# ChenWu98/cycle-diffusion

Measured on NVIDIA H100. Metric: images/sec (512x512, 50-step encode+decode) at 1/2/4/8 H100; ms/U-Net-call, higher is better.
Workload: dtype fp32

## Files before the change

cycle_diffusion_b200/_cabi.py:

```python
import ctypes as C
import os

HERE = os.path.dirname(os.path.abspath(__file__))
LIB_PATH = os.path.join(HERE, 'libcdx.so')

CDX_UNET_OPENAI = 1
CDX_UNET_IDDPM = 2
CDX_UNET_DDPM = 3
CDX_TEXT_OPENCLIP = 4
CDX_PRED_EPS = 0
CDX_PRED_V = 1


class UnetConfig(C.Structure):
    _fields_ = [('kind', C.c_int), ('in_channels', C.c_int), ('out_channels', C.c_int), ('model_channels', C.c_int),
                ('num_res_blocks', C.c_int), ('n_mult', C.c_int), ('channel_mult', C.c_int * 8), ('n_attn', C.c_int),
                ('attention_ds', C.c_int * 8), ('num_heads', C.c_int), ('num_head_channels', C.c_int),
                ('context_dim', C.c_int)]


class VaeConfig(C.Structure):
    _fields_ = [('ch', C.c_int), ('n_mult', C.c_int), ('ch_mult', C.c_int * 8), ('num_res_blocks', C.c_int),
                ('in_channels', C.c_int), ('out_ch', C.c_int), ('z_channels', C.c_int), ('embed_dim', C.c_int), ('vq', C.c_int), ('n_embed', C.c_int)]

# ... 99 lines not shown

class SemanticAttnMaskC(C.Structure):
    _fields_ = [('intersect', C.c_int), ('n_tokens', C.c_int * CDX_SEMANTIC_MAX)]


class LocalBlendC(C.Structure):
    _fields_ = [('alpha_src', C.c_void_p), ('alpha_tgt', C.c_void_p), ('sub_src', C.c_void_p), ('sub_tgt', C.c_void_p), ('start_step', C.c_int),
                ('th_blend', C.c_float), ('th_sub', C.c_float)]


_F = C.c_float
_I = C.c_int
_S = C.c_size_t

SIGNATURES = {
    'cdx_abi_version': (_I, []),
    'cdx_last_error': (C.c_char_p, []),
    'cdx_engine_create': (_I, [_I, C.POINTER(_P)]),
    'cdx_engine_destroy': (None, [_P]),
    'cdx_engine_workspace_bytes': (_S, [_P]),
    'cdx_engine_launch_count': (C.c_uint64, [_P]),
    'cdx_engine_set_mma_mode': (_I, [_P, _I]),
    'cdx_engine_set_persist': (_I, [_P, _I, _I]),
    'cdx_engine_profile': (_I, [_P, _I]),
    'cdx_engine_profile_read': (_I, [_P, _I, C.POINTER(C.c_double), C.POINTER(C.c_double), C.POINTER(C.c_double), C.POINTER(C.c_uint64)]),
    'cdx_unet_create': (_I, [_P, C.POINTER(UnetConfig), C.POINTER(_P)]),
    'cdx_vae_create': (_I, [_P, C.POINTER(VaeConfig), C.POINTER(_P)]),
    'cdx_text_create': (_I, [_P, C.POINTER(TextConfig), C.POINTER(_P)]),
    'cdx_net_destroy': (None, [_P]),
    'cdx_net_num_params': (_I, [_P]),
    'cdx_net_param_name': (C.c_char_p, [_P, _I]),
    'cdx_net_param_shape': (_I, [_P, _I, C.POINTER(C.c_int64)]),
    'cdx_net_load_param': (_I, [_P, C.c_char_p, _P, _I, C.POINTER(C.c_int64), _I]),
    'cdx_net_finalize': (_I, [_P]),
    'cdx_net_weight_blob': (_I, [_P, C.POINTER(_P), C.POINTER(_S)]),
    'cdx_net_adopt_blob': (_I, [_P]),
    'cdx_unet_set_time_freqs': (_I, [_P, C.POINTER(_F), _I]),
    'cdx_unet_set_prediction': (_I, [_P, _I, C.POINTER(_F), C.POINTER(_F), _I]),
    'cdx_unet_forward': (_I, [_P, _P, _P, _P, _I, _P, _I, _I, _I, _P]),
    'cdx_vae_encode': (_I, [_P, _P, _P, _I, _I, _P]),
    'cdx_text_encode': (_I, [_P, _P, _I, _I, _P, _P]),
    'cdx_vae_decode': (_I, [_P, _P, _P, _I, _I, _P]),
    'cdx_vae_encode_hw': (_I, [_P, _P, _P, _I, _I, _I, _P]),
    'cdx_vae_decode_hw': (_I, [_P, _P, _P, _I, _I, _I, _P]),
    'cdx_affine': (_I, [_P, _P, _F, _F, _P, _S, _P]),
    'cdx_shift_scale': (_I, [_P, _P, _F, _F, _P, _S, _P]),
# ... 108 lines not shown
```

cycle_diffusion_b200/csrc/cabi.cu:

```cuda
#include <stdio.h>
#include <stdlib.h>
#include <string.h>

#include <algorithm>

#include "nets.cuh"

struct cdx_engine { cdx::Engine e; };
struct cdx_net { cdx::Net* n; cdx_engine* owner; };

namespace cdx {
const std::string& last_error();

namespace {

template <class F>
int guard(F&& f) {
  try {
    f();
    return CDX_OK;
  } catch (const Error& err) {
    set_last_error(err.what());
    return err.code;
  } catch (const std::exception& err) {
// ... 569 lines not shown

int cdx_abi_version(void) { return CDX_ABI_VERSION; }
const char* cdx_last_error(void) { return cdx::last_error().c_str(); }

int cdx_engine_create(int device, cdx_engine** out) {
  return guard([&] {
    CDX_CHECK(out != nullptr, "engine_create: null out");
    int count = 0;
    cudaError_t err = cudaGetDeviceCount(&count);
    if (err != cudaSuccess || count <= 0)
      throw Error(CDX_E_CUDA, std::string("no usable CUDA device (there is no CPU fallback): ") + cudaGetErrorString(err));
    CDX_CHECK(device >= 0 && device < count, "engine_create: device %d out of range (count %d)", device, count);
    CDX_CUDA(cudaSetDevice(device));
    cudaDeviceProp prop;
    CDX_CUDA(cudaGetDeviceProperties(&prop, device));
    cdx_engine* eng = new cdx_engine();
    eng->e.device = device;
    if (prop.major != 9 || prop.minor != 0)
      throw Error(CDX_E_CUDA, "libcdx is built for sm_90a (H100) only; device " + std::to_string(device) + " is sm_" +
                                  std::to_string(prop.major) + std::to_string(prop.minor));
    eng->e.num_sms = prop.multiProcessorCount;
    const char* persist = getenv("CDX_PERSIST");
    eng->e.persist = persist == nullptr || atoi(persist) != 0;
    *out = eng;
  });
}
void cdx_engine_destroy(cdx_engine* e) {
  if (!e) return;
  cudaSetDevice(e->e.device);
  cudaDeviceSynchronize();
  e->e.arena.destroy();
  if (e->e.done_ev) cudaEventDestroy(e->e.done_ev);
  if (e->e.side) cudaStreamDestroy(e->e.side);
  if (e->e.fork_ev) cudaEventDestroy(e->e.fork_ev);
  if (e->e.join_ev) cudaEventDestroy(e->e.join_ev);
  if (e->e.amax_pool) cudaFree(e->e.amax_pool);
  delete e;
}
size_t cdx_engine_workspace_bytes(const cdx_engine* e) { return e ? e->e.arena.cap : 0; }
uint64_t cdx_engine_launch_count(const cdx_engine* e) { return e ? e->e.launches : 0; }
int cdx_engine_set_mma_mode(cdx_engine* e, int mode) {
  return guard([&] {
    CDX_CHECK(e != nullptr && mode >= 0 && mode <= 5, "set_mma_mode: bad arguments");
    e->e.mma_mode = mode == 0 ? 0 : 1;
    e->e.flash_attn = mode != 2 && mode != 0;
    e->e.tc_kind = mode == 3 ? 0 : mode >= 4 ? 2 : 1;
    e->e.attn_one = mode == 5;
  });
}

int cdx_engine_set_persist(cdx_engine* e, int enable, int max_ctas) {
  return guard([&] {
    CDX_CHECK(e != nullptr && max_ctas >= 0, "set_persist: bad arguments");
    e->e.persist = enable != 0;
    e->e.persist_grid = max_ctas;
  });
}

int cdx_engine_profile(cdx_engine* e, int enable) {
  return guard([&] {
    CDX_CHECK(e != nullptr, "profile: null engine");
    CDX_CUDA(cudaSetDevice(e->e.device));
    CDX_CUDA(cudaDeviceSynchronize());
    for (ProfRec& r : e->e.prof.recs) { cudaEventDestroy(r.a); cudaEventDestroy(r.b); }
    e->e.prof.recs.clear();
    e->e.prof.on = enable != 0;
  });
}
int cdx_engine_profile_read(cdx_engine* e, int tag, double* ms, double* flops, double* bytes, uint64_t* launches) {
  return guard([&] {
    CDX_CHECK(e && ms && flops && bytes && launches && tag >= 0 && tag < PROF_NTAGS, "profile_read: bad arguments");
    CDX_CUDA(cudaSetDevice(e->e.device));
    CDX_CUDA(cudaDeviceSynchronize());
    *ms = 0; *flops = 0; *bytes = 0; *launches = 0;
    const bool dump = getenv("CDX_PROF_DUMP") != nullptr;
    for (const ProfRec& r : e->e.prof.recs) {
      if (r.tag != tag) continue;
      float t = 0.f;
// ... 1226 lines not shown
```

cycle_diffusion_b200/csrc/common.cuh:

```cuda
#pragma once
#include <cuda_runtime.h>
#include <stdint.h>
#include <stdio.h>
#include <string>
#include <vector>
#include <stdexcept>

#include "../../include/cdx.h"

namespace cdx {

struct Error : std::runtime_error {
  int code;
  Error(int c, const std::string& m) : std::runtime_error(m), code(c) {}
};
void set_last_error(const std::string& m);

#define CDX_CHECK(cond, ...)                                                     \
  do {                                                                           \
    if (!(cond)) {                                                               \
      char _b[512];                                                              \
      snprintf(_b, sizeof(_b), __VA_ARGS__);                                     \
      throw ::cdx::Error(CDX_E_INVALID, std::string(_b) + " [" #cond "]");       \
    }                                                                            \
// ... 22 lines not shown
};

enum ProfTag {
  PROF_CONV_FFMA = 0, PROF_DENSE_FFMA = 1, PROF_BATCHED_FFMA = 2, PROF_CONV_TC = 3, PROF_DENSE_TC = 4, PROF_BATCHED_TC = 5,
  PROF_GROUPNORM = 6, PROF_LAYERNORM = 7, PROF_SOFTMAX = 8, PROF_ELEMENTWISE = 9, PROF_NTAGS = 10
};
struct ProfRec { cudaEvent_t a, b; int tag; double flops, bytes; int launches; char note[56]; };
struct Profiler {
  bool on = false;
  std::vector<ProfRec> recs;
  std::vector<cudaEvent_t> pool;
};

struct Engine {
  Profiler prof;
  int device = 0;
  int num_sms = 132;
  bool flash_attn = true;
  int mma_mode = 1;
  int tc_kind = 1;
  bool attn_one = false;
  bool persist = true;
  int persist_grid = 0;
  float* amax_pool = nullptr;
  int amax_cap = 1 << 15, amax_used = 0, amax_high = 0;
  float* amax_slot();
  double* stat_pool = nullptr;
  size_t stat_cap = (size_t)8 << 20, stat_used = 0, stat_high = 0;
  size_t stat_dry = 0;
  double* stat_alloc(size_t n);
  void pools_reset(cudaStream_t s);
  Arena arena;
  cudaStream_t last_stream = nullptr;
  cudaEvent_t done_ev = nullptr;
  bool ev_recorded = false;
  cudaStream_t side = nullptr;
  cudaEvent_t fork_ev = nullptr, join_ev = nullptr;
  uint64_t launches = 0;
  bool dry() const { return arena.dry; }
};

struct ProfScope {
  Engine& e;
  cudaStream_t s;
  int idx = -1;
  ProfScope(Engine& eng, cudaStream_t st, int tag, double flops, double bytes, int launches);
// ... 32 lines not shown
  const float* Bw = nullptr; int ldb = 0; int b_kn = 0;
  const float* Bw_hi = nullptr; const float* Bw_lo = nullptr;
  const void* Bw_h_hi = nullptr; const void* Bw_h_lo = nullptr; int b_exp = 0;
  const float* a_amax = nullptr; const float* a2_amax = nullptr;
  float* c_amax = nullptr;
  double* c_stats = nullptr;
  float* Cout = nullptr; int ldc = 0;
  float* Cout_lo = nullptr;
  float* Ct_hi = nullptr; float* Ct_lo = nullptr; int t_col0 = 0; long long ldt = 0;
  const float* bias = nullptr;
  const float* rowvec = nullptr; int ld_rowvec = 0; int rows_per_batch = 1;
  const float* residual = nullptr; int ldr = 0;
  float alpha = 1.f;
  int geglu = 0;
  int out_nchw = 0;
  int rows_per_img = 0;
  int batch = 1, heads = 1;
  long long sA_b = 0, sA_h = 0, sB_b = 0, sB_h = 0, sC_b = 0, sC_h = 0;
};
void gemm(Engine& e, const GemmArgs& a, cudaStream_t s, int* route = nullptr);
bool gemm_tc(Engine& e, const GemmArgs& a, cudaStream_t s, int* side_done = nullptr);
enum { ROUTE_KIND_SS = 0, ROUTE_KIND_TS = 1, ROUTE_KIND_H16 = 2, ROUTE_KIND_H16_FAST = 3 };
inline int route_plan(int kind, int width, int splits) { return kind << 4 | width << 8 | splits << 16; }
bool flash_eligible(const Engine& e, int N, int Nk, int d, int C);
struct AttnPlanes {
  enum Fmt { TF32, H16 } fmt;
  const void* q_hi; const void* q_lo; int ldq;
  const void* k_hi; const void* k_lo; int ldk;
  const void* vt_hi; const void* vt_lo;
  const float* q_amax = nullptr; const float* k_amax = nullptr; const float* v_amax = nullptr;
};
bool flash_attention(Engine& e, const AttnPlanes& a, float* out, int ldo, int B, int N, int Nk, int Nks, int Nvs, int heads, int d, float scale,
                     cudaStream_t s, const int* qk_row = nullptr, const int* acc_rows = nullptr, int n_acc = 0, const int* kv_row = nullptr);
void split_rows_h16(Engine& e, const float* src, long long rows, int cols, long long ld, void* hi, void* lo, long long ldh, const float* amax,
                    cudaStream_t s);
void split_transpose_h16(Engine& e, const float* src, int R, int Cc, long long ld, void* hi, void* lo, const float* amax, cudaStream_t s,
                         int images = 1, int Rp = 0);
struct FlashPlan { int qrows, rag, ksplit, ring; };
FlashPlan flash_plan(int d, bool h16, bool one, int N);
bool self_attention_h16(Engine& e, const float* qkv, const float* slot, float* out, int B, int HW, int C, int heads, int d, float scale, bool lo,
                        cudaStream_t s, const int* qk_row, const int* kv_row, const int* acc_rows = nullptr, int n_acc = 0, int* Nvs_out = nullptr);
bool self_attention_tf32_padded(Engine& e, const float* qk_hi, const float* qk_lo, const float* vr, float* out, int B, int HW, int C, int heads,
                                int d, float scale, cudaStream_t s, const int* qk_row, const int* kv_row, const int* acc_rows = nullptr,
                                int n_acc = 0, int* Nvs_out = nullptr);
void context_split_h16(Engine& e, const float* kv, int Mk, int C, const float* slot, void* k_hi, void* k_lo, void* vt_hi, void* vt_lo,
                       cudaStream_t s);
// ... 127 lines not shown
```

cycle_diffusion_b200/csrc/kernels_tc.cu:

```cuda
#include <algorithm>

#include <mutex>
#include <array>
#include <map>
#include <unordered_map>
#include <vector>
#include <cstdlib>
#include <cmath>
#include <type_traits>

#include <cuda_fp16.h>

#include "tc_common.cuh"

namespace cdx {
namespace {

using namespace tc;

constexpr int TBM = 128, TBN = 128, TBK = 32;
constexpr int TILE_BYTES = TBM * TBK * 4;
constexpr int TC_THREADS = 384;
constexpr int SMEM_MAX = 232448;
constexpr int BAR_BYTES = 256, ALIGN_SLACK = 1024;
// ... 93 lines not shown
  } else {
    c.m0 = tm * TBM;
    c.zb = z / p.heads;
    c.zh = z - c.zb * p.heads;
  }
  return c;
}

__device__ __forceinline__ uint32_t tf32_lo(float x, uint32_t hi) { return rn_tf32(__float_as_uint(x - __uint_as_float(hi))); }

#ifdef CDX_GEMM_TIMELINE
constexpr int TL_SLOTS = 8;
__device__ unsigned long long* g_gemm_timeline = nullptr;
__device__ __forceinline__ void tl_stamp(int k) {
  unsigned long long t;
  asm volatile("mov.u64 %0, %%globaltimer;" : "=l"(t) :: "memory");
  if (g_gemm_timeline) g_gemm_timeline[(size_t)blockIdx.x * TL_SLOTS + k] = t;
}
#define TL_STAMP(k) tl_stamp(k)
#else
#define TL_STAMP(k) ((void)0)
#endif

template <int KIND, int BN, bool PERSIST = false>
__global__ void __launch_bounds__(TC_THREADS, 1)
tc_gemm_kernel(const __grid_constant__ CUtensorMap mapA, const __grid_constant__ CUtensorMap mapA2,
               const __grid_constant__ CUtensorMap mapB, const __grid_constant__ CUtensorMap mapBlo,
               const __grid_constant__ CUtensorMap mapR, const __grid_constant__ CUtensorMap mapC, const TcParams p) {
  using CF = Cfg<KIND, BN, PERSIST>;
  constexpr bool H16 = CF::H16, FAST = KIND == KIND_H16_FAST;
  constexpr int BK = CF::BK, KSTEPS = CF::KSTEPS, A_BYTES = CF::A_BYTES, B_PLANE = CF::B_PLANE, STAGE_BYTES = CF::STAGE_BYTES;
  constexpr int STAGES = CF::STAGES, EPI_BOX = CF::EPI_BOX, EPI_PER_SLOT = CF::EPI_PER_SLOT, EPI_SLOTS = CF::EPI_SLOTS;
  constexpr int NACC = BN / 2;
  if (threadIdx.x == 0) TL_STAMP(0);
  pdl_trigger();
  extern __shared__ uint8_t smem_raw[];
  const uint32_t base = (smem_u32(smem_raw) + 1023u) & ~1023u;
  const uint32_t epi = base + STAGES * STAGE_BYTES;
  const uint32_t bars = epi + CF::EPI_BYTES;
  auto bar_full = [&](int s) { return bars + 8u * s; };
  auto bar_empty = [&](int s) { return bars + 8u * (STAGES + s); };
  const uint32_t bar_res = bars + 16u * STAGES;
  const uint32_t bar_out = bar_res + 8u;

  const int warp = threadIdx.x >> 5, lane = threadIdx.x & 31;
  const int num_kb = (p.K + BK - 1) / BK;
  TileCoord tc_ = tile_coord(p, blockIdx.x, num_kb);
  int nst = tc_.kb1 - tc_.kb0;
  const bool staged = PERSIST || staged_store(p);
  auto epi_box = [&](int k) {
    return PERSIST ? epi + k * EPI_BOX : base + ((nst + k / EPI_PER_SLOT) % STAGES) * STAGE_BYTES + (k % EPI_PER_SLOT) * EPI_BOX;
  };

  if (threadIdx.x == 0) {
    for (int s = 0; s < STAGES; ++s) {
      mbar_init(bar_full(s), 1);
// ... 64 lines not shown
    asm volatile("setmaxnreg.dec.sync.aligned.u32 40;");
    if (threadIdx.x == 0) {
      const int cblocks = p.mode == 1 ? p.C1 / TBK : 0;
      int it = 0;
      for (int kb = tc_.kb0; kb < tc_.kb1; ++kb, ++it) {
        const int s = it % STAGES;
        mbar_wait(bar_empty(s), ((it / STAGES) & 1) ^ 1);
        const uint32_t st = base + s * STAGE_BYTES;
        const uint32_t sb = st + A_BYTES;
        const int k0 = kb * BK;
        if (p.mode == 2) {
          mbar_expect_tx(bar_full(s), TILE_BYTES + BN * 128);
          int ca[4], cb4[4];
#pragma unroll
          for (int i = 0; i < 4; ++i) {
            const int ac = p.a_code[i], bc = p.b_code[i];
            ca[i] = ac == 0 ? k0 : ac == 1 ? tc_.m0 + tc_.zh * p.a_rowoff_h : ac == 2 ? tc_.zh : ac == 3 ? tc_.zb : 0;
            cb4[i] = bc == 0 ? k0 : bc == 1 ? tc_.n0 + tc_.zh * p.b_rowoff_h : bc == 2 ? tc_.zh : bc == 3 ? tc_.zb : 0;
          }
          tma_load_4d(st, &mapA, ca[0], ca[1], ca[2], ca[3], bar_full(s));
          tma_load_4d(sb, &mapB, cb4[0], cb4[1], cb4[2], cb4[3], bar_full(s));
          continue;
        }
        mbar_expect_tx(bar_full(s), TILE_BYTES + (KIND == KIND_SS ? 1 : 2) * B_PLANE);
        if (p.mode == 0) {
          if (k0 < p.C1) tma_load_2d(st, &mapA, k0, tc_.m0, bar_full(s));
          else tma_load_2d(st, &mapA2, k0 - p.C1, tc_.m0, bar_full(s));
        } else {
          const int tap = kb / cblocks, cb = kb - tap * cblocks;
          const int dy = tap / 3, dx = tap - dy * 3;
          tma_load_4d(st, &mapA, cb * TBK, tc_.x0 * p.cstride + dx - p.cpad, tc_.y0 * p.cstride + dy - p.cpad, tc_.b0,
                      bar_full(s));
        }
        tma_load_2d(sb, &mapB, k0, tc_.n0, bar_full(s));
        if (KIND != KIND_SS) tma_load_2d(sb + B_PLANE, &mapBlo, k0, tc_.n0, bar_full(s));
      }
      if (staged) {
        if (p.residual) mbar_expect_tx(bar_res, BN * TBM * 4);
        for (int k = 0; k < EPI_SLOTS; ++k, ++it) {
          const int s = it % STAGES;
          mbar_wait(bar_empty(s), ((it / STAGES) & 1) ^ 1);
          if (!p.residual) continue;
          for (int b = k * EPI_PER_SLOT; b < min(BN / TBK, (k + 1) * EPI_PER_SLOT); ++b) {
            const uint32_t dst = epi_box(b);
            if (p.mode == 0) tma_load_2d(dst, &mapR, tc_.n0 + b * TBK, tc_.m0, bar_res);
            else tma_load_4d(dst, &mapR, tc_.n0 + b * TBK, tc_.x0, tc_.y0, tc_.b0, bar_res);
          }
        }
        if (!p.residual) mbar_arrive(bar_res);
      }
    }
    return;
  }

  asm volatile("setmaxnreg.inc.sync.aligned.u32 232;");
// ... 5 lines not shown
  float omax_cta = 0.f;
  int g0 = 0;
#pragma unroll 1
  for (int t = blockIdx.x, item = 0;;) {
    const int kchunk = (tc_.kb1 - tc_.kb0) <= 2 * CF::KCHUNK ? 2 * CF::KCHUNK : CF::KCHUNK;
    int px[2] = {0, 0}, py[2] = {0, 0}, pb[2] = {0, 0};
    if (p.mode == 1) {
#pragma unroll
      for (int i = 0; i < 2; ++i) {
        const int r = r0 + 8 * i;
        px[i] = tc_.x0 + r % p.bw; py[i] = tc_.y0 + (r / p.bw) % p.bh; pb[i] = tc_.b0 + r / (p.bw * p.bh);
      }
    }

    float acc[NACC], tot[NACC];
#pragma unroll
    for (int j = 0; j < NACC; ++j) { acc[j] = 0.f; tot[j] = 0.f; }

    struct Frag { uint32_t h[KSTEPS][4], l[KSTEPS][4]; };

    auto load_split = [&](int it, Frag& f) {
      const int s = (g0 + it) % STAGES;
      mbar_wait(bar_full(s), ((g0 + it) / STAGES) & 1);
      const uint32_t st = base + s * STAGE_BYTES;
      if (KIND == KIND_SS) {
        const uint32_t sb = st + A_BYTES;
        const int ct = threadIdx.x - 128;
#pragma unroll 4
        for (int i = ct; i < B_PLANE / 16; i += 256) {
          const uint32_t a = sb + (uint32_t)i * 16u;
          uint32_t v[4], h[4], l[4];
          asm volatile("ld.shared.v4.u32 {%0, %1, %2, %3}, [%4];" : "=r"(v[0]), "=r"(v[1]), "=r"(v[2]), "=r"(v[3]) : "r"(a));
#pragma unroll
          for (int c = 0; c < 4; ++c) { h[c] = rn_tf32(v[c]); l[c] = tf32_lo(__uint_as_float(v[c]), h[c]); }
          asm volatile("st.shared.v4.u32 [%0], {%1, %2, %3, %4};" ::"r"(a), "r"(h[0]), "r"(h[1]), "r"(h[2]), "r"(h[3]) : "memory");
          asm volatile("st.shared.v4.u32 [%0], {%1, %2, %3, %4};" ::"r"(a + B_PLANE), "r"(l[0]), "r"(l[1]), "r"(l[2]), "r"(l[3]) : "memory");
        }
        asm volatile("fence.proxy.async.shared::cta;" ::: "memory");
        asm volatile("bar.sync 1, 256;" ::: "memory");
      }
#pragma unroll
      for (int kk = 0; kk < KSTEPS; ++kk) {
        if (H16) {
#pragma unroll
          for (int i = 0; i < 2; ++i) {
            const int r = r0 + 8 * i;
// ... 13 lines not shown
              }
            }
          }
        } else {
#pragma unroll
          for (int i = 0; i < 2; ++i) {
            const int r = r0 + 8 * i;
#pragma unroll
            for (int hk = 0; hk < 2; ++hk) {
              const int k = kk * 8 + hk * 4 + qd;
              float x;
              asm volatile("ld.shared.f32 %0, [%1];" : "=f"(x)
                           : "r"(st + (uint32_t)r * 128u + ((((uint32_t)k >> 2) ^ (uint32_t)(r & 7)) << 4) + (uint32_t)(k & 3) * 4u));
              const uint32_t h = rn_tf32(__float_as_uint(x));
              f.h[kk][hk * 2 + i] = h;
              f.l[kk][hk * 2 + i] = tf32_lo(x, h);
            }
          }
        }
      }
    };

    auto mma = [&](int it, const Frag& f) {
      const uint32_t sb = base + ((g0 + it) % STAGES) * STAGE_BYTES + A_BYTES;
      const uint64_t bhi = H16 ? make_desc_sw64(sb) : make_desc(sb), blo = H16 ? make_desc_sw64(sb + B_PLANE) : make_desc(sb + B_PLANE);
      wgmma_pin(acc);
      wgmma_fence();
#pragma unroll
      for (int kk = 0; kk < KSTEPS; ++kk) {
        const uint64_t adv = (uint64_t)kk * 2u;
        if (H16) {
          if (!FAST) {
            Wgmma<BN>::f16_rs(acc, f.l[kk], bhi + adv);
            Wgmma<BN>::f16_rs(acc, f.h[kk], blo + adv);
          }
          Wgmma<BN>::f16_rs(acc, f.h[kk], bhi + adv);
        } else {
          Wgmma<BN>::tf32_rs(acc, f.l[kk], bhi + adv);
          Wgmma<BN>::tf32_rs(acc, f.h[kk], blo + adv);
          Wgmma<BN>::tf32_rs(acc, f.h[kk], bhi + adv);
        }
      }
      wgmma_commit();
    };

    int kin = 0;
    auto step = [&](int it, const Frag& cur, Frag& nxt) {
      mma(it, cur);
      wgmma_wait1();
      if (it > 0) {
        __syncwarp();
        if (lane == 0) mbar_arrive(bar_empty((g0 + it - 1) % STAGES));
      }
      if (it + 1 < nst) load_split(it + 1, nxt);
// ... 263 lines not shown
  for (long long i = (long long)blockIdx.x * blockDim.x + threadIdx.x; i < total; i += (long long)gridDim.x * blockDim.x) {
    const long long r = i / c4n;
    const int c4 = (int)(i - r * c4n);
    const float4 v = *reinterpret_cast<const float4*>(x + r * ld + 4 * c4);
    m = fmaxf(m, fmaxf(fmaxf(fabsf(v.x), fabsf(v.y)), fmaxf(fabsf(v.z), fabsf(v.w))));
  }
#pragma unroll
  for (int o = 16; o > 0; o >>= 1) m = fmaxf(m, __shfl_xor_sync(0xffffffffu, m, o));
  if ((threadIdx.x & 31) == 0) atomicMax(reinterpret_cast<unsigned int*>(slot), __float_as_uint(m));
}

__global__ void amax_rows_scalar_kernel(const float* __restrict__ x, long long rows, int C, long long ld, float* __restrict__ slot) {
  float m = 0.f;
  const long long total = rows * (long long)C;
  for (long long i = (long long)blockIdx.x * blockDim.x + threadIdx.x; i < total; i += (long long)gridDim.x * blockDim.x) {
    const long long r = i / C;
    m = fmaxf(m, fabsf(x[r * ld + (i - r * C)]));
  }
#pragma unroll
  for (int o = 16; o > 0; o >>= 1) m = fmaxf(m, __shfl_xor_sync(0xffffffffu, m, o));
  if ((threadIdx.x & 31) == 0) atomicMax(reinterpret_cast<unsigned int*>(slot), __float_as_uint(m));
}

template <int KIND, int BN, bool PERSIST = false>
void set_smem_attr() {
  CDX_CUDA(cudaFuncSetAttribute(tc_gemm_kernel<KIND, BN, PERSIST>, cudaFuncAttributeMaxDynamicSharedMemorySize, Cfg<KIND, BN, PERSIST>::SMEM_BYTES));
}

void ensure_attr(int device) {
  static bool attr_set[64] = {};
  static std::mutex mtx;
  std::lock_guard<std::mutex> lock(mtx);
  const int d = device & 63;
  if (!attr_set[d]) {
    set_smem_attr<KIND_SS, 128>();
    set_smem_attr<KIND_TS, 128>();
    set_smem_attr<KIND_TS, 64>();
    set_smem_attr<KIND_H16, 128>();
    set_smem_attr<KIND_H16, 64>();
    set_smem_attr<KIND_H16_FAST, 128>();
    set_smem_attr<KIND_H16_FAST, 64>();
    set_smem_attr<KIND_H16, 128, true>();
    set_smem_attr<KIND_H16, 64, true>();
    set_smem_attr<KIND_H16_FAST, 128, true>();
    set_smem_attr<KIND_H16_FAST, 64, true>();
    attr_set[d] = true;
  }
}

template <int KIND, int BN>
void launch_gemm(const TcParams& p, const CUtensorMap& mA, const CUtensorMap& mA2, const CUtensorMap& mB, const CUtensorMap& mBlo,
                 const CUtensorMap& mR, const CUtensorMap& mC, cudaStream_t s) {
  launch_ex(tc_gemm_kernel<KIND, BN>, dim3((unsigned)p.total_tiles), dim3(TC_THREADS), Cfg<KIND, BN>::SMEM_BYTES, s, 1, mA, mA2, mB, mBlo, mR, mC, p);
}

template <int KIND, int BN>
void launch_gemm_persist(const TcParams& p, int ctas, const CUtensorMap& mA, const CUtensorMap& mA2, const CUtensorMap& mB,
                         const CUtensorMap& mBlo, const CUtensorMap& mR, const CUtensorMap& mC, cudaStream_t s) {
  launch_ex(tc_gemm_kernel<KIND, BN, true>, dim3((unsigned)ctas), dim3(TC_THREADS), Cfg<KIND, BN, true>::SMEM_BYTES, s, 1, mA, mA2, mB, mBlo, mR, mC, p);
}

}

void split_planes(Engine& e, const float* w, float* hi, float* lo, size_t n, cudaStream_t s) {
  if (e.dry()) return;
  size_t blocks = (n + 255) / 256;
  if (blocks > (size_t)e.num_sms * 16) blocks = (size_t)e.num_sms * 16;
  split_planes_kernel<<<(unsigned)(blocks ? blocks : 1), 256, 0, s>>>(w, hi, lo, n);
  CDX_CUDA(cudaGetLastError());
  e.launches++;
}

void split_planes_h16(Engine& e, const float* w, void* hi, void* lo, size_t n, int exp, cudaStream_t s) {
  if (e.dry()) return;
  size_t blocks = (n + 255) / 256;
  if (blocks > (size_t)e.num_sms * 16) blocks = (size_t)e.num_sms * 16;
// ... 223 lines not shown
  p.kb_per_split = cdiv(num_kb, best_s);
  p.splits = cdiv(num_kb, p.kb_per_split);
  p.kb_per_split *= bk / TBK;
  p.total_tiles = tiles * p.splits;
  Scope ws_scope(e.arena);
  if (p.splits > 1) p.ws = (float*)e.arena.alloc((size_t)p.splits * a.M * a.N * sizeof(float));
  if (h16) {
    p.a_amax = a.a_amax;
    p.a2_amax = a.A2 ? a.a2_amax : nullptr;
    if (!p.a_amax) {
      float* slot = e.amax_slot();
      if (a.mode == 1) amax_rows(e, a.A, (long long)(a.M / (a.Hout * a.Wout)) * a.Hin * a.Win, a.C1, a.lda, slot, s);
      else amax_rows(e, a.A, a.M, a.C1, a.lda, slot, s);
      p.a_amax = slot;
    }
    if (a.A2 && !p.a2_amax) {
      float* slot = e.amax_slot();
      amax_rows(e, a.A2, a.M, a.C2, a.lda2, slot, s);
      p.a2_amax = slot;
    }
    p.b_exp = a.b_exp;
  }
  const bool fast = h16 && e.tc_kind == 2;
  p.c_amax = a.out_nchw ? nullptr : a.c_amax;
  const bool quad_ok = a.mode == 1 ? ((p.bw * p.bh) % 32 == 0 && p.tiles_x * p.bw == p.W && p.tiles_y * p.bh == p.H) : (a.rows_per_batch % 32 == 0);
  p.c_stats = (a.c_stats && quad_ok && p.splits == 1 && !a.out_nchw && !a.geglu && !a.Ct_hi && !a.Cout_lo && a.ldc == a.N) ? a.c_stats : nullptr;
  if (side_done)
    *side_done = (p.c_amax ? 1 : 0) | (p.c_stats ? 2 : 0) | (p.splits > 1 ? 4 : 0) |
                 route_plan(fast ? ROUTE_KIND_H16_FAST : h16 ? ROUTE_KIND_H16 : ts ? ROUTE_KIND_TS : ROUTE_KIND_SS, p.tn_w, p.splits);
  if (e.dry()) return true;
  if (h16) {
    uint64_t d[2] = {(uint64_t)a.K, (uint64_t)a.N}, st[1] = {(uint64_t)a.ldb * 2};
    uint32_t bx[2] = {(uint32_t)TBK, (uint32_t)p.tn_w};
    mB = &get_map(a.Bw_h_hi, 2, d, st, bx, nullptr, 2, 64);
    mBlo = &get_map(a.Bw_h_lo, 2, d, st, bx, nullptr, 2, 64);
  } else {
    uint64_t d[2] = {(uint64_t)a.K, (uint64_t)a.N}, st[1] = {(uint64_t)a.ldb * 4};
    uint32_t bx[2] = {TBK, (uint32_t)p.tn_w};
    mB = &get_map(ts ? a.Bw_hi : a.Bw, 2, d, st, bx);
    mBlo = ts ? &get_map(a.Bw_lo, 2, d, st, bx) : mB;
  }
  const CUtensorMap *mR = mA, *mC = mA;
  if (staged_store(p)) {
    auto out_map = [&](const float* ptr, int cols, int ld) -> const CUtensorMap& {
      if (a.mode == 0) {
        uint64_t d[2] = {(uint64_t)cols, (uint64_t)a.M}, st[1] = {(uint64_t)ld * 4};
        uint32_t bx[2] = {TBK, TBM};
        return get_map(ptr, 2, d, st, bx);
      }
      uint64_t d[4] = {(uint64_t)cols, (uint64_t)p.W, (uint64_t)p.H, (uint64_t)p.B};
      uint64_t st[3] = {(uint64_t)ld * 4, (uint64_t)ld * 4 * p.W, (uint64_t)ld * 4 * p.W * p.H};
      uint32_t bx[4] = {TBK, (uint32_t)p.bw, (uint32_t)p.bh, (uint32_t)p.bn};
      return get_map(ptr, 4, d, st, bx);
    };
    mC = &out_map(a.Cout, a.geglu ? a.N / 2 : a.N, a.ldc);
    if (a.residual) mR = &out_map(a.residual, a.N, a.ldr);
  }
  ensure_attr(e.device);
  ProfScope ps(e, s, a.mode == 1 ? PROF_CONV_TC : PROF_DENSE_TC, 2.0 * a.M * a.N * a.K,
               4.0 * ((double)a.M * a.K / (a.mode == 1 ? 9 : 1) + (double)a.N * a.K + (double)a.M * a.N), 1);
  ps.note("M%d N%d K%d w%d tiles%d S%d %s%s%s%s%s box%dx%dx%d", a.M, a.N, a.K, p.tn_w, tiles, p.splits, h16 ? (fast ? "H16x1" : "H16") : ts ? "TS" : "SS",
          a.Cout_lo ? " planes" : "", a.geglu ? " geglu" : "", a.residual ? " res" : "", persist_ok && staged_store(p) ? " persist" : "", p.bw, p.bh, p.bn);
  const bool persist = persist_ok && staged_store(p);
  const int ctas = (int)std::min<long long>(p.total_tiles, e.persist_grid > 0 ? std::min(e.persist_grid, e.num_sms) : e.num_sms);
  if (persist && fast && p.tn_w == 128) launch_gemm_persist<KIND_H16_FAST, 128>(p, ctas, *mA, *mA2, *mB, *mBlo, *mR, *mC, s);
  else if (persist && fast) launch_gemm_persist<KIND_H16_FAST, 64>(p, ctas, *mA, *mA2, *mB, *mBlo, *mR, *mC, s);
  else if (persist && p.tn_w == 128) launch_gemm_persist<KIND_H16, 128>(p, ctas, *mA, *mA2, *mB, *mBlo, *mR, *mC, s);
  else if (persist) launch_gemm_persist<KIND_H16, 64>(p, ctas, *mA, *mA2, *mB, *mBlo, *mR, *mC, s);
  else if (fast && p.tn_w == 128) launch_gemm<KIND_H16_FAST, 128>(p, *mA, *mA2, *mB, *mBlo, *mR, *mC, s);
  else if (fast) launch_gemm<KIND_H16_FAST, 64>(p, *mA, *mA2, *mB, *mBlo, *mR, *mC, s);
  else if (h16 && p.tn_w == 128) launch_gemm<KIND_H16, 128>(p, *mA, *mA2, *mB, *mBlo, *mR, *mC, s);
  else if (h16) launch_gemm<KIND_H16, 64>(p, *mA, *mA2, *mB, *mBlo, *mR, *mC, s);
  else if (ts && p.tn_w == 128) launch_gemm<KIND_TS, 128>(p, *mA, *mA2, *mB, *mBlo, *mR, *mC, s);
  else if (ts) launch_gemm<KIND_TS, 64>(p, *mA, *mA2, *mB, *mBlo, *mR, *mC, s);
  else launch_gemm<KIND_SS, 128>(p, *mA, *mA2, *mB, *mBlo, *mR, *mC, s);
  CDX_CUDA(cudaGetLastError());
  e.launches++;
  if (p.splits > 1) {
    const long long total4 = (long long)a.M * a.N / 4;
    const int blocks = (int)std::min<long long>((total4 + 255) / 256, (long long)e.num_sms * 8);
    launch_ex(splitk_reduce_kernel, dim3((unsigned)blocks), dim3(256), 0, s, 1, p.ws, p.splits, p, h16 ? 1 : 0);
    CDX_CUDA(cudaGetLastError());
    e.launches++;
  }
  return true;
}

}
// ... 7 lines not shown
```

cycle_diffusion_b200/engine.py:

```python
import contextlib
import ctypes as C
import math

import torch

from . import _cabi
from ._cabi import lib, check, UnetConfig, VaeConfig, TextConfig, DdimCoef, PixelCoef
from .attn_control import LocalBlend, MutualSelfControl, PnPControl
from .schedule import EditFriendlySchedule
from .semantic import SemanticGuidance


def _ptr(t):
    return C.c_void_p(t.data_ptr()) if t is not None else C.c_void_p(0)


def _f32c(t, device):
    assert t.dtype == torch.float32, f'expected float32, got {t.dtype}'
    if t.device != device:
        t = t.to(device)
    return t.contiguous()


def check_mask(mask, shape, device, what='mask'):
# ... 27 lines not shown
        try:
            self.close()
        except Exception:
            pass

    @property
    def stream(self):
        return C.c_void_p(torch.cuda.current_stream(self.device).cuda_stream)

    @property
    def launches(self):
        return int(lib.cdx_engine_launch_count(self.h))

    @property
    def workspace_bytes(self):
        return int(lib.cdx_engine_workspace_bytes(self.h))

    def set_mma_mode(self, mode):
        check(lib.cdx_engine_set_mma_mode(self.h, int(mode)))
        self.mma_mode = int(mode)

    def set_persist(self, enable, max_ctas=0):
        check(lib.cdx_engine_set_persist(self.h, int(bool(enable)), int(max_ctas)))

    PRECISIONS = {'full': None, 'autocast': 5}

    @contextlib.contextmanager
    def precision(self, precision):
        if precision not in self.PRECISIONS:
            raise ValueError(f'precision must be one of {sorted(self.PRECISIONS)}, got {precision!r}')
        mode, prev = self.PRECISIONS[precision], self.mma_mode
        if mode is None:
            yield self
            return
        self.set_mma_mode(mode)
        try:
            yield self
        finally:
            self.set_mma_mode(prev)

    PROF_TAGS = ['conv3x3_ffma', 'dense_ffma', 'batched_ffma', 'conv3x3_tc', 'dense_tc', 'batched_tc', 'groupnorm', 'layernorm',
                 'softmax', 'other']

    def profile(self, enable):
        check(lib.cdx_engine_profile(self.h, int(enable)))

# ... 258 lines not shown
                                      eps, _ptr(y), _ptr(amax), _ptr(stats), _ptr(yn), C.byref(path), self.stream))
        return y, amax, stats, yn, self.PRODUCE_PATHS[path.value]

    GEMM_POINTERS = ('A', 'A2', 'w', 'bias', 'rowvec', 'residual', 'C', 'C_lo', 'Ct_hi', 'Ct_lo', 'a_amax', 'a2_amax', 'c_amax', 'c_stats')
    GEMM_KINDS = ('ss', 'ts', 'h16', 'h16_fast')

    def op_gemm(self, **fields):
        d = _cabi.GemmDesc(alpha=1.0, stride=1, pad=1, batch=1, heads=1, rows_per_batch=1, up=1)
        for name, v in fields.items():
            if name in self.GEMM_POINTERS:
                if v is not None:
                    want = torch.float64 if name == 'c_stats' else torch.float32
                    assert torch.is_tensor(v) and v.dtype == want and v.device == self.device, f'op_gemm: {name} must be a {want} tensor on {self.device}'
                setattr(d, name, v.data_ptr() if v is not None else None)
            else:
                assert hasattr(d, name), f'op_gemm: no field {name}'
                setattr(d, name, v)
        plan = C.c_int(0)
        check(lib.cdx_op_gemm(self.h, C.byref(d), C.byref(plan), self.stream))
        return self.gemm_plan(plan.value)

    @classmethod
    def gemm_plan(cls, p):
        return dict(kind=cls.GEMM_KINDS[(p >> 4) & 3] if p & 8 else 'ffma', width=(p >> 8) & 255, splits=(p >> 16) & 255,
                    amax_fused=bool(p & 1), stats_fused=bool(p & 2))

    def op_latent_chains(self, stage, chains, chw, n_src, K, rows, c=None, cnext=None, **fields):
        sg_rows = fields.pop('sg_rows', None)
        m = len(sg_rows) // max(n_src * K, 1) if sg_rows else 0
        hw = fields.get('hw', 0)
        need = dict(x0=n_src * chw, noise0=n_src * chw, xt=n_src * chw, xn=n_src * chw, noise_next=n_src * chw, xn2=n_src * chw,
                    eout=rows * chw, xin=rows * chw, yt=n_src * K * chw, y_out=n_src * K * chw,
                    z_out=(n_src - 1) * fields.get('z_stride', 0) + chw, eps_in=(n_src - 1) * fields.get('eps_stride', 0) + chw,
                    mask=n_src * hw, sg_thr=n_src * K * m * ((chw // hw if hw else 0) if not fields.get('sg_mask') else 2),
                    sg_nu=n_src * K * chw, sg_map=n_src * K * m * fields.get('sg_gh', 0) * fields.get('sg_gw', 0), d_src=n_src * chw,
                    d_tgt=n_src * K * chw)
        assert len(chains) == n_src * (1 + K), f'op_latent_chains: {len(chains)} chains for n_src={n_src}, K={K}'
        table = (_cabi.LatentChain * len(chains))(*[_cabi.LatentChain(int(r), int(r2), float(s)) for r, r2, s in chains])
        d = _cabi.LatentChainsSamplerDesc(chw=chw, n_src=n_src, K=K, rows=rows, chains=table)
        if sg_rows:
            assert len(sg_rows) == n_src * K * m, f'op_latent_chains: {len(sg_rows)} concept rows for {n_src * K} target chains'
            sg_table = (C.c_int * len(sg_rows))(*[int(r) for r in sg_rows])
            d.sg_m, d.sg_rows = m, sg_table
        for name in ('sg_scale', 'sg_lambda'):
            if name in fields:
                vals = [float(v) for v in fields.pop(name)]
                setattr(d, name, (C.c_float * 8)(*(vals + [0.0] * (8 - len(vals)))))
        if c is not None:
# ... 613 lines not shown
```

include/cdx.h:

```cpp
#ifndef CDX_H_
#define CDX_H_

#include <stddef.h>
#include <stdint.h>

#ifdef __cplusplus
extern "C" {
#endif

#define CDX_ABI_VERSION 2

#define CDX_OK 0
#define CDX_E_INVALID (-1)
#define CDX_E_CUDA (-2)
#define CDX_E_STATE (-3)
#define CDX_E_NOMEM (-4)

typedef struct cdx_engine cdx_engine;
typedef struct cdx_net cdx_net;

int cdx_abi_version(void);
const char* cdx_last_error(void);
int cdx_engine_create(int device, cdx_engine** out);
void cdx_engine_destroy(cdx_engine* e);
size_t cdx_engine_workspace_bytes(const cdx_engine* e);
uint64_t cdx_engine_launch_count(const cdx_engine* e);
#define CDX_PROF_NTAGS 10
int cdx_engine_profile(cdx_engine* e, int enable);
int cdx_engine_profile_read(cdx_engine* e, int tag, double* ms, double* flops, double* bytes, uint64_t* launches);
int cdx_engine_set_mma_mode(cdx_engine* e, int mode);
int cdx_engine_set_persist(cdx_engine* e, int enable, int max_ctas);

#define CDX_UNET_OPENAI 1
#define CDX_UNET_IDDPM 2
#define CDX_UNET_DDPM 3

typedef struct cdx_unet_config {
  int kind;
  int in_channels, out_channels, model_channels, num_res_blocks;
  int n_mult;
  int channel_mult[8];
  int n_attn;
  int attention_ds[8];
  int num_heads;
  int num_head_channels;
  int context_dim;
} cdx_unet_config;

typedef struct cdx_vae_config {
  int ch;
  int n_mult;
  int ch_mult[8];
  int num_res_blocks;
  int in_channels, out_ch, z_channels, embed_dim;
// ... 362 lines not shown
```

Measured before the change: 0.9002.

## Pre-split conv activations into fp16 hi/lo planes for SS wgmma A operand

For implicit-GEMM 3x3 convs on the fp16 split path with N>=128, the activation is first split once into fp16 hi/lo planes in the arena. The kernel then TMA-loads both planes into shared memory and uses shared-memory-descriptor wgmma for A, skipping the per-k-step register fragment split. This removes repeated split work inside the GEMM (each input pixel is read by up to 9 taps) but adds a separate split pass, extra workspace, and drops the persistent-kernel path for these convs. The route is on by default and can be disabled with an env var or API call.

```diff
diff --git a/cycle_diffusion_b200/_cabi.py b/cycle_diffusion_b200/_cabi.py
--- a/cycle_diffusion_b200/_cabi.py
+++ b/cycle_diffusion_b200/_cabi.py
@@ -145,6 +145,7 @@
     'cdx_engine_launch_count': (C.c_uint64, [_P]),
     'cdx_engine_set_mma_mode': (_I, [_P, _I]),
     'cdx_engine_set_persist': (_I, [_P, _I, _I]),
+    'cdx_engine_set_conv_planes': (_I, [_P, _I]),
     'cdx_engine_profile': (_I, [_P, _I]),
     'cdx_engine_profile_read': (_I, [_P, _I, C.POINTER(C.c_double), C.POINTER(C.c_double), C.POINTER(C.c_double), C.POINTER(C.c_uint64)]),
     'cdx_unet_create': (_I, [_P, C.POINTER(UnetConfig), C.POINTER(_P)]),
diff --git a/cycle_diffusion_b200/csrc/cabi.cu b/cycle_diffusion_b200/csrc/cabi.cu
--- a/cycle_diffusion_b200/csrc/cabi.cu
+++ b/cycle_diffusion_b200/csrc/cabi.cu
@@ -615,6 +615,8 @@
     eng->e.num_sms = prop.multiProcessorCount;
     const char* persist = getenv("CDX_PERSIST");
     eng->e.persist = persist == nullptr || atoi(persist) != 0;
+    const char* conv_planes = getenv("CDX_CONV_PLANES");
+    eng->e.conv_planes = conv_planes == nullptr || atoi(conv_planes) != 0;
     *out = eng;
   });
 }
@@ -647,6 +649,13 @@
     CDX_CHECK(e != nullptr && max_ctas >= 0, "set_persist: bad arguments");
     e->e.persist = enable != 0;
     e->e.persist_grid = max_ctas;
+  });
+}
+
+int cdx_engine_set_conv_planes(cdx_engine* e, int enable) {
+  return guard([&] {
+    CDX_CHECK(e != nullptr, "set_conv_planes: null engine");
+    e->e.conv_planes = enable != 0;
   });
 }
 
diff --git a/cycle_diffusion_b200/csrc/common.cuh b/cycle_diffusion_b200/csrc/common.cuh
--- a/cycle_diffusion_b200/csrc/common.cuh
+++ b/cycle_diffusion_b200/csrc/common.cuh
@@ -68,6 +68,7 @@
   bool attn_one = false;
   bool persist = true;
   int persist_grid = 0;
+  bool conv_planes = true;
   float* amax_pool = nullptr;
   int amax_cap = 1 << 15, amax_used = 0, amax_high = 0;
   float* amax_slot();
@@ -146,6 +147,8 @@
 bool gemm_tc(Engine& e, const GemmArgs& a, cudaStream_t s, int* side_done = nullptr);
 enum { ROUTE_KIND_SS = 0, ROUTE_KIND_TS = 1, ROUTE_KIND_H16 = 2, ROUTE_KIND_H16_FAST = 3 };
 inline int route_plan(int kind, int width, int splits) { return kind << 4 | width << 8 | splits << 16; }
+enum { ROUTE_A_PLANES = 64 };
+inline bool conv_planes_route(bool on, bool h16, int mode, int N) { return on && h16 && mode == 1 && N >= 128; }
 bool flash_eligible(const Engine& e, int N, int Nk, int d, int C);
 struct AttnPlanes {
   enum Fmt { TF32, H16 } fmt;
diff --git a/cycle_diffusion_b200/csrc/kernels_tc.cu b/cycle_diffusion_b200/csrc/kernels_tc.cu
--- a/cycle_diffusion_b200/csrc/kernels_tc.cu
+++ b/cycle_diffusion_b200/csrc/kernels_tc.cu
@@ -139,7 +139,7 @@
 #define TL_STAMP(k) ((void)0)
 #endif
 
-template <int KIND, int BN, bool PERSIST = false>
+template <int KIND, int BN, bool PERSIST = false, bool PLANES = false>
 __global__ void __launch_bounds__(TC_THREADS, 1)
 tc_gemm_kernel(const __grid_constant__ CUtensorMap mapA, const __grid_constant__ CUtensorMap mapA2,
                const __grid_constant__ CUtensorMap mapB, const __grid_constant__ CUtensorMap mapBlo,
@@ -149,6 +149,8 @@
   constexpr int BK = CF::BK, KSTEPS = CF::KSTEPS, A_BYTES = CF::A_BYTES, B_PLANE = CF::B_PLANE, STAGE_BYTES = CF::STAGE_BYTES;
   constexpr int STAGES = CF::STAGES, EPI_BOX = CF::EPI_BOX, EPI_PER_SLOT = CF::EPI_PER_SLOT, EPI_SLOTS = CF::EPI_SLOTS;
   constexpr int NACC = BN / 2;
+  static_assert(!PLANES || (H16 && !PERSIST), "planes-A: fp16 split, one CTA per work item");
+  constexpr int A_PLANE = A_BYTES / 2;
   if (threadIdx.x == 0) TL_STAMP(0);
   pdl_trigger();
   extern __shared__ uint8_t smem_raw[];
@@ -259,15 +261,16 @@
           tma_load_4d(sb, &mapB, cb4[0], cb4[1], cb4[2], cb4[3], bar_full(s));
           continue;
         }
-        mbar_expect_tx(bar_full(s), TILE_BYTES + (KIND == KIND_SS ? 1 : 2) * B_PLANE);
+        mbar_expect_tx(bar_full(s), (PLANES && FAST ? A_PLANE : TILE_BYTES) + (KIND == KIND_SS ? 1 : 2) * B_PLANE);
         if (p.mode == 0) {
           if (k0 < p.C1) tma_load_2d(st, &mapA, k0, tc_.m0, bar_full(s));
           else tma_load_2d(st, &mapA2, k0 - p.C1, tc_.m0, bar_full(s));
         } else {
           const int tap = kb / cblocks, cb = kb - tap * cblocks;
           const int dy = tap / 3, dx = tap - dy * 3;
-          tma_load_4d(st, &mapA, cb * TBK, tc_.x0 * p.cstride + dx - p.cpad, tc_.y0 * p.cstride + dy - p.cpad, tc_.b0,
-                      bar_full(s));
+          const int cx = tc_.x0 * p.cstride + dx - p.cpad, cy = tc_.y0 * p.cstride + dy - p.cpad;
+          tma_load_4d(st, &mapA, cb * TBK, cx, cy, tc_.b0, bar_full(s));
+          if (PLANES && !FAST) tma_load_4d(st + A_PLANE, &mapA2, cb * TBK, cx, cy, tc_.b0, bar_full(s));
         }
         tma_load_2d(sb, &mapB, k0, tc_.n0, bar_full(s));
         if (KIND != KIND_SS) tma_load_2d(sb + B_PLANE, &mapBlo, k0, tc_.n0, bar_full(s));
@@ -319,6 +322,7 @@
     auto load_split = [&](int it, Frag& f) {
       const int s = (g0 + it) % STAGES;
       mbar_wait(bar_full(s), ((g0 + it) / STAGES) & 1);
+      if (PLANES) return;
       const uint32_t st = base + s * STAGE_BYTES;
       if (KIND == KIND_SS) {
         const uint32_t sb = st + A_BYTES;
@@ -378,14 +382,21 @@
     };
 
     auto mma = [&](int it, const Frag& f) {
-      const uint32_t sb = base + ((g0 + it) % STAGES) * STAGE_BYTES + A_BYTES;
+      const uint32_t sa = base + ((g0 + it) % STAGES) * STAGE_BYTES, sb = sa + A_BYTES;
       const uint64_t bhi = H16 ? make_desc_sw64(sb) : make_desc(sb), blo = H16 ? make_desc_sw64(sb + B_PLANE) : make_desc(sb + B_PLANE);
+      const uint64_t ahi = make_desc_sw64(sa + (uint32_t)wg * 4096u), alo = make_desc_sw64(sa + A_PLANE + (uint32_t)wg * 4096u);
       wgmma_pin(acc);
       wgmma_fence();
 #pragma unroll
       for (int kk = 0; kk < KSTEPS; ++kk) {
         const uint64_t adv = (uint64_t)kk * 2u;
-        if (H16) {
+        if (PLANES) {
+          if (!FAST) {
+            Wgmma<BN>::f16_ss(acc, alo + adv, bhi + adv);
+            Wgmma<BN>::f16_ss(acc, ahi + adv, blo + adv);
+          }
+          Wgmma<BN>::f16_ss(acc, ahi + adv, bhi + adv);
+        } else if (H16) {
           if (!FAST) {
             Wgmma<BN>::f16_rs(acc, f.l[kk], bhi + adv);
             Wgmma<BN>::f16_rs(acc, f.h[kk], blo + adv);
@@ -695,9 +706,9 @@
   if ((threadIdx.x & 31) == 0) atomicMax(reinterpret_cast<unsigned int*>(slot), __float_as_uint(m));
 }
 
-template <int KIND, int BN, bool PERSIST = false>
+template <int KIND, int BN, bool PERSIST = false, bool PLANES = false>
 void set_smem_attr() {
-  CDX_CUDA(cudaFuncSetAttribute(tc_gemm_kernel<KIND, BN, PERSIST>, cudaFuncAttributeMaxDynamicSharedMemorySize, Cfg<KIND, BN, PERSIST>::SMEM_BYTES));
+  CDX_CUDA(cudaFuncSetAttribute(tc_gemm_kernel<KIND, BN, PERSIST, PLANES>, cudaFuncAttributeMaxDynamicSharedMemorySize, Cfg<KIND, BN, PERSIST>::SMEM_BYTES));
 }
 
 void ensure_attr(int device) {
@@ -717,14 +728,18 @@
     set_smem_attr<KIND_H16, 64, true>();
     set_smem_attr<KIND_H16_FAST, 128, true>();
     set_smem_attr<KIND_H16_FAST, 64, true>();
+    set_smem_attr<KIND_H16, 128, false, true>();
+    set_smem_attr<KIND_H16, 64, false, true>();
+    set_smem_attr<KIND_H16_FAST, 128, false, true>();
+    set_smem_attr<KIND_H16_FAST, 64, false, true>();
     attr_set[d] = true;
   }
 }
 
-template <int KIND, int BN>
+template <int KIND, int BN, bool PLANES = false>
 void launch_gemm(const TcParams& p, const CUtensorMap& mA, const CUtensorMap& mA2, const CUtensorMap& mB, const CUtensorMap& mBlo,
                  const CUtensorMap& mR, const CUtensorMap& mC, cudaStream_t s) {
-  launch_ex(tc_gemm_kernel<KIND, BN>, dim3((unsigned)p.total_tiles), dim3(TC_THREADS), Cfg<KIND, BN>::SMEM_BYTES, s, 1, mA, mA2, mB, mBlo, mR, mC, p);
+  launch_ex(tc_gemm_kernel<KIND, BN, false, PLANES>, dim3((unsigned)p.total_tiles), dim3(TC_THREADS), Cfg<KIND, BN>::SMEM_BYTES, s, 1, mA, mA2, mB, mBlo, mR, mC, p);
 }
 
 template <int KIND, int BN>
@@ -994,13 +1009,29 @@
     p.b_exp = a.b_exp;
   }
   const bool fast = h16 && e.tc_kind == 2;
+  const bool planes = conv_planes_route(e.conv_planes, h16, a.mode, a.N);
+  void *a_hi = nullptr, *a_lo = nullptr;
+  const long long a_pix = planes ? (long long)p.B * a.Hin * a.Win : 0;
+  if (planes) {
+    a_hi = e.arena.alloc((size_t)a_pix * a.C1 * 2);
+    if (!fast) a_lo = e.arena.alloc((size_t)a_pix * a.C1 * 2);
+  }
   p.c_amax = a.out_nchw ? nullptr : a.c_amax;
   const bool quad_ok = a.mode == 1 ? ((p.bw * p.bh) % 32 == 0 && p.tiles_x * p.bw == p.W && p.tiles_y * p.bh == p.H) : (a.rows_per_batch % 32 == 0);
   p.c_stats = (a.c_stats && quad_ok && p.splits == 1 && !a.out_nchw && !a.geglu && !a.Ct_hi && !a.Cout_lo && a.ldc == a.N) ? a.c_stats : nullptr;
   if (side_done)
     *side_done = (p.c_amax ? 1 : 0) | (p.c_stats ? 2 : 0) | (p.splits > 1 ? 4 : 0) |
-                 route_plan(fast ? ROUTE_KIND_H16_FAST : h16 ? ROUTE_KIND_H16 : ts ? ROUTE_KIND_TS : ROUTE_KIND_SS, p.tn_w, p.splits);
+                 route_plan(fast ? ROUTE_KIND_H16_FAST : h16 ? ROUTE_KIND_H16 : ts ? ROUTE_KIND_TS : ROUTE_KIND_SS, p.tn_w, p.splits) |
+                 (planes ? ROUTE_A_PLANES : 0);
   if (e.dry()) return true;
+  if (planes) {
+    uint64_t d[4] = {(uint64_t)a.C1, (uint64_t)a.Win, (uint64_t)a.Hin, (uint64_t)p.B};
+    uint64_t st[3] = {(uint64_t)a.C1 * 2, (uint64_t)a.C1 * 2 * a.Win, (uint64_t)a.C1 * 2 * a.Win * a.Hin};
+    uint32_t bx[4] = {TBK, (uint32_t)(p.bw * a.stride), (uint32_t)(p.bh * a.stride), (uint32_t)p.bn};
+    uint32_t es[4] = {1, (uint32_t)a.stride, (uint32_t)a.stride, 1};
+    mA = &get_map(a_hi, 4, d, st, bx, es, 2, 64);
+    mA2 = fast ? mA : &get_map(a_lo, 4, d, st, bx, es, 2, 64);
+  }
   if (h16) {
     uint64_t d[2] = {(uint64_t)a.K, (uint64_t)a.N}, st[1] = {(uint64_t)a.ldb * 2};
     uint32_t bx[2] = {(uint32_t)TBK, (uint32_t)p.tn_w};
@@ -1032,10 +1063,15 @@
   ProfScope ps(e, s, a.mode == 1 ? PROF_CONV_TC : PROF_DENSE_TC, 2.0 * a.M * a.N * a.K,
                4.0 * ((double)a.M * a.K / (a.mode == 1 ? 9 : 1) + (double)a.N * a.K + (double)a.M * a.N), 1);
   ps.note("M%d N%d K%d w%d tiles%d S%d %s%s%s%s%s box%dx%dx%d", a.M, a.N, a.K, p.tn_w, tiles, p.splits, h16 ? (fast ? "H16x1" : "H16") : ts ? "TS" : "SS",
-          a.Cout_lo ? " planes" : "", a.geglu ? " geglu" : "", a.residual ? " res" : "", persist_ok && staged_store(p) ? " persist" : "", p.bw, p.bh, p.bn);
+          a.Cout_lo ? " planes" : planes ? " A-planes" : "", a.geglu ? " geglu" : "", a.residual ? " res" : "", persist_ok && staged_store(p) ? " persist" : "", p.bw, p.bh, p.bn);
+  if (planes) split_rows_h16(e, a.A, a_pix, a.C1, a.lda, a_hi, a_lo, a.C1, p.a_amax, s);
   const bool persist = persist_ok && staged_store(p);
   const int ctas = (int)std::min<long long>(p.total_tiles, e.persist_grid > 0 ? std::min(e.persist_grid, e.num_sms) : e.num_sms);
-  if (persist && fast && p.tn_w == 128) launch_gemm_persist<KIND_H16_FAST, 128>(p, ctas, *mA, *mA2, *mB, *mBlo, *mR, *mC, s);
+  if (planes && fast && p.tn_w == 128) launch_gemm<KIND_H16_FAST, 128, true>(p, *mA, *mA2, *mB, *mBlo, *mR, *mC, s);
+  else if (planes && fast) launch_gemm<KIND_H16_FAST, 64, true>(p, *mA, *mA2, *mB, *mBlo, *mR, *mC, s);
+  else if (planes && p.tn_w == 128) launch_gemm<KIND_H16, 128, true>(p, *mA, *mA2, *mB, *mBlo, *mR, *mC, s);
+  else if (planes) launch_gemm<KIND_H16, 64, true>(p, *mA, *mA2, *mB, *mBlo, *mR, *mC, s);
+  else if (persist && fast && p.tn_w == 128) launch_gemm_persist<KIND_H16_FAST, 128>(p, ctas, *mA, *mA2, *mB, *mBlo, *mR, *mC, s);
   else if (persist && fast) launch_gemm_persist<KIND_H16_FAST, 64>(p, ctas, *mA, *mA2, *mB, *mBlo, *mR, *mC, s);
   else if (persist && p.tn_w == 128) launch_gemm_persist<KIND_H16, 128>(p, ctas, *mA, *mA2, *mB, *mBlo, *mR, *mC, s);
   else if (persist) launch_gemm_persist<KIND_H16, 64>(p, ctas, *mA, *mA2, *mB, *mBlo, *mR, *mC, s);
diff --git a/cycle_diffusion_b200/engine.py b/cycle_diffusion_b200/engine.py
--- a/cycle_diffusion_b200/engine.py
+++ b/cycle_diffusion_b200/engine.py
@@ -73,6 +73,9 @@
 
     def set_persist(self, enable, max_ctas=0):
         check(lib.cdx_engine_set_persist(self.h, int(bool(enable)), int(max_ctas)))
+
+    def set_conv_planes(self, enable):
+        check(lib.cdx_engine_set_conv_planes(self.h, int(bool(enable))))
 
     PRECISIONS = {'full': None, 'autocast': 5}
 
@@ -377,8 +380,11 @@
 
     @classmethod
     def gemm_plan(cls, p):
-        return dict(kind=cls.GEMM_KINDS[(p >> 4) & 3] if p & 8 else 'ffma', width=(p >> 8) & 255, splits=(p >> 16) & 255,
+        plan = dict(kind=cls.GEMM_KINDS[(p >> 4) & 3] if p & 8 else 'ffma', width=(p >> 8) & 255, splits=(p >> 16) & 255,
                     amax_fused=bool(p & 1), stats_fused=bool(p & 2))
+        if p & 64:
+            plan['a_planes'] = True
+        return plan
 
     def op_latent_chains(self, stage, chains, chw, n_src, K, rows, c=None, cnext=None, **fields):
         sg_rows = fields.pop('sg_rows', None)
diff --git a/include/cdx.h b/include/cdx.h
--- a/include/cdx.h
+++ b/include/cdx.h
@@ -30,6 +30,7 @@
 int cdx_engine_profile_read(cdx_engine* e, int tag, double* ms, double* flops, double* bytes, uint64_t* launches);
 int cdx_engine_set_mma_mode(cdx_engine* e, int mode);
 int cdx_engine_set_persist(cdx_engine* e, int enable, int max_ctas);
+int cdx_engine_set_conv_planes(cdx_engine* e, int enable);
 
 #define CDX_UNET_OPENAI 1
 #define CDX_UNET_IDDPM 2
```

Result: faster. 0.9095, median of 6 (+1.0%).
